# mgp25/OpenLTE

Measured on AMD Instinct MI355X. Metric: DL subframes/sec @20MHz 100RB 64QAM, full chain FFT->CE->demap->rate-unmatch->turbo(REF)->CRC (SURVEY 8d W4), higher is better.
Workload: dtype i8 IQ in, f32 FFT/CE/equaliser, i8 soft bits, i16 path metrics (differences exact modulo 2^16); 1 GPU; W4 full DL chain: 20 MHz/100 RB/64QAM, 9 allocations per subframe (8x12 PRB TBS 3240 + 1x4 PRB TBS 1064), 65536 subframes per GPU, int8 IQ in HBM; subframes_per_gpu=65536, N_ant=1, CFI=2, channel_estimate_form=compact, decoder=REF (reference-faithful, bit-exact), unique_subframes=96, streams_per_gpu=1

## Files before the change

openlte_amd/csrc/turbo.hip:

```cpp
#include <algorithm>
#include <cstring>
#include <initializer_list>
#include <type_traits>
#include <vector>

#include "plan_core.hpp"
#include "turbo_swar.h"

using namespace turbo_geom;

namespace {

constexpr uint32_t RX_NULL_AS_INT = 10000;


__device__ __forceinline__ int sbyte(uint32_t w, int k) { return (int)__builtin_amdgcn_sbfe(w, 8 * k, 8); }

typedef __attribute__((address_space(3))) const uint8_t  lds_u8_t;
typedef __attribute__((address_space(3))) const int8_t   lds_i8_t;
typedef __attribute__((address_space(3))) const uint16_t lds_u16_t;
__device__ __forceinline__ uint32_t lds_u8(uint32_t addr) { return *(lds_u8_t *)(uintptr_t)addr; }
__device__ __forceinline__ int      lds_i8(uint32_t addr) { return *(lds_i8_t *)(uintptr_t)addr; }
__device__ __forceinline__ uint32_t lds_u16(uint32_t addr) { return *(lds_u16_t *)(uintptr_t)addr; }

// ... 967 lines not shown
            }
            if (t < n_t) {
                const uint32_t w = (ch * 64 + t) >> 5, left = n_t - t;
                for (; t < n_t; t += 8) steps8(t);
                decw[(gi * n_w32 + w) * 4 + j] = accv << (32u - left);
            }
        }
        __syncthreads();
    }

#ifdef SMALL_PAD
    if ((padv[0] ^ padv[1] ^ padv[2] ^ padv[3]) == 0x12345678u) decw[0] = 0;
#endif
    uint32_t cur = 0;
    {
        const uint32_t q0 = (uint32_t)__builtin_amdgcn_mov_dpp((int)XY, 0x00, 0xF, 0xF, false), q1 = (uint32_t)__builtin_amdgcn_mov_dpp((int)XY, 0x55, 0xF, 0xF, false);
        const uint32_t q2 = (uint32_t)__builtin_amdgcn_mov_dpp((int)XY, 0xAA, 0xF, 0xF, false), q3 = (uint32_t)__builtin_amdgcn_mov_dpp((int)XY, 0xFF, 0xF, 0xF, false);
        const short pm[8] = {(short)q0, (short)q1, (short)q2, (short)q3, (short)(q0 >> 16), (short)(q1 >> 16), (short)(q2 >> 16), (short)(q3 >> 16)};
        int best = 0;
#pragma unroll
        for (int st = 1; st < 8; st++) {
            const int d = (short)(pm[st] - pm[0]);
            if (d < best) { best = d; cur = st; }
        }
    }

    const uint2 MAP_ID = make_uint2(0x03020100u, 0x07060504u);
    for (uint32_t g = 0; g < n_g; g++) {
        uint32_t       end = (uint32_t)__builtin_amdgcn_readlane((int)cur, (int)(g * 4));
        const uint32_t cb  = mode ? (T0 + g) >> 1 : T0 + g;
        uint32_t      *sgn = pass_of(g).sgn + (seg_off >> 5) + ((size_t)(cb >> 6) * n_chunk * 64 + (cb & 63u)) * 2;
        for (int ch = (int)n_chunk - 1; ch >= 0; ch--) {
            const uint32_t t = (uint32_t)ch * 64 + lane;
            const uint4    w = *reinterpret_cast<const uint4 *>(&decw[(g * n_w32 + (t >> 5)) * 4]);
            const uint32_t sh = 31u - (t & 31u);
            uint2          G = MAP_ID;
            if (t < K) {
                const uint32_t f = 0x06040200u + (((w.x >> sh) & 1u) | ((w.y >> sh) & 1u) << 8 | ((w.z >> sh) & 1u) << 16 | ((w.w >> sh) & 1u) << 24);
                G = make_uint2(f, f);
            }
            G = map_compose(G, map_row_shl<1>(G, MAP_ID));
            G = map_compose(G, map_row_shl<2>(G, MAP_ID));
            G = map_compose(G, map_row_shl<4>(G, MAP_ID));
            G = map_compose(G, map_row_shl<8>(G, MAP_ID));
            const uint32_t row = lane >> 4;
#pragma unroll
            for (int r = 1; r < 4; r++) {
                const uint2 R = make_uint2((uint32_t)__builtin_amdgcn_readlane((int)G.x, 16 * r), (uint32_t)__builtin_amdgcn_readlane((int)G.y, 16 * r));
                if (row < (uint32_t)r) G = map_compose(G, R);
            }
            const uint2    Gn  = make_uint2((uint32_t)__shfl_down((int)G.x, 1u), (uint32_t)__shfl_down((int)G.y, 1u));
            const uint32_t nxt = lane == 63 ? end : map_at(Gn, end);
            const uint32_t st  = map_at(G, end);
            const bool     pos = (nxt < st) || (nxt == st && nxt == 0);
            const uint64_t neg = __ballot(t < K && !pos);
            if (lane == 0) *reinterpret_cast<uint2 *>(sgn + (size_t)ch * 64 * 2) = make_uint2((uint32_t)neg, (uint32_t)(neg >> 32));
            end = (uint32_t)__builtin_amdgcn_readlane((int)st, 0);
        }
    }
}

namespace sw = turbo_swar;
struct UnitWords { uint32_t w[5]; };
__device__ __forceinline__ UnitWords load_unit_words(const uint8_t *arr, size_t tile_off, uint32_t lane, uint32_t u)
{
    const uint4 c    = *reinterpret_cast<const uint4 *>(arr + unit_off(tile_off, lane, u));
    uint32_t    prev = 0x7F7F7F7Fu;
    if (u > 0) prev = *reinterpret_cast<const uint32_t *>(arr + unit_off(tile_off, lane, u - 1) + 12);
    return UnitWords{{prev, c.x, c.y, c.z, c.w}};
}
__device__ __forceinline__ UnitWords load_unit_joined(const uint8_t *mag, const uint32_t *sgn, size_t tile_off, uint32_t lane, uint32_t u)
{
    UnitWords      w = load_unit_words(mag, tile_off, lane, u);
    const uint32_t *sp = sgn + (tile_off >> 5) + ((size_t)(u >> 2) * 64 + lane) * 2;
    const uint2    c = *reinterpret_cast<const uint2 *>(sp);
    uint32_t       ph = 0;
    if ((u & 3u) == 0 && u > 0) ph = sp[1 - 128];
    const uint32_t b = sw::unit_sign_bits(c.x, c.y, ph, u);
    if (u > 0) w.w[0] = sw::joined_from_bits(w.w[0], b & 15u);
#pragma unroll
    for (int j = 0; j < 4; j++) w.w[j + 1] = sw::joined_from_bits(w.w[j + 1], (b >> (4 * j + 4)) & 15u);
    return w;
}
struct PermArgs { const uint8_t *M1; const uint32_t *S1;  const uint8_t *X2; uint8_t *out[2];  };

#ifndef PERM_NB
#define PERM_NB 4
#endif
static_assert(PERM_NB == PERM_BLOCKS, "a size's perm grid is a multiple of 128 workgroups (the merged decode's map granularity) only for four blocks per workgroup");
template <int NSLOT, bool MULTI = false>
__global__ __launch_bounds__(384) void k_turbo_perm(PermArgs a, uint32_t K_arg, uint32_t n_cb_arg, const uint16_t *__restrict__ pi_arg, MultiArgs ma)
{
    static_assert(NSLOT == 1, "one unit per thread");
    uint32_t K = K_arg, n_cb = n_cb_arg, bidx = blockIdx.x, grid = gridDim.x;
    size_t   seg_off = 0;
    const uint16_t *__restrict__ pi = pi_arg;
    if constexpr (MULTI) {
        const_seg_t &sg = multi_seg(ma, blockIdx.x >> 7);
        K = sg.K; n_cb = sg.n_cb; pi = (const uint16_t *)sg.pi; bidx = blockIdx.x - sg.wg_perm; grid = sg.perm_grid;
        seg_off = sg.arr_off;
    }
    extern __shared__ __attribute__((aligned(16))) int8_t smp[];
    int8_t *mtab = smp, *sm = smp + MTAB_N;
    const uint32_t Kp = kpad64(K), n_units = Kp >> 4;
    int           *red_i = reinterpret_cast<int *>(sm + Kp);
    const uint32_t u0 = threadIdx.x;
    const int      nv = (u0 < n_units) ? min(16, max(0, (int)K - 16 * (int)u0)) : -1;
    IdxRaw         praw;
    {
        const uint4 *ip = reinterpret_cast<const uint4 *>(pi + 16 * (size_t)(nv > 0 ? u0 : 0));
        const uint32_t kk = K | K << 16;
        praw.lo = ip[0];
        praw.hi = (nv > 8) ? ip[1] : make_uint4(kk, kk, kk, kk);
    }
#pragma unroll 1
    for (uint32_t it = 0; it < PERM_NB; it++) {
        const uint32_t cb = xcd_cb(bidx + it * grid, n_cb), tile = cb >> 6, lane = cb & 63;
        const size_t   tile_off = seg_off + (size_t)tile * Kp * 64;
        if (cb >= n_cb) {
            if (MULTI && cb < ((n_cb + 63u) & ~63u) && nv >= 0) {
                *reinterpret_cast<uint4 *>(a.out[0] + unit_off(tile_off, lane, u0)) = make_uint4(0, 0, 0, 0);
                *reinterpret_cast<uint4 *>(a.out[1] + unit_off(tile_off, lane, u0)) = make_uint4(0, 0, 0, 0);
            }
            continue;
        }
        uint32_t u = u0;
        asm volatile("" : "+v"(u), "+v"(praw.lo.x), "+v"(praw.lo.y), "+v"(praw.lo.z), "+v"(praw.lo.w), "+v"(praw.hi.x), "+v"(praw.hi.y), "+v"(praw.hi.z), "+v"(praw.hi.w));
        uint4          X2 = make_uint4(0, 0, 0, 0);
        if (nv >= 0) {
            const UnitWords wa = load_unit_joined(a.M1, a.S1, tile_off, lane, u);
            uint32_t        pa = wa.w[0];
            X2 = *reinterpret_cast<const uint4 *>(a.X2 + unit_off(tile_off, lane, u));
            uint32_t c1[4];
#pragma unroll
            for (int j = 0; j < 4; j++) {
                const uint32_t ja = wa.w[j + 1];
                const sw::SM4  A  = sw::unjoin(ja);
                c1[j] = (4 * j < nv) ? sw::to_tc(sw::step3(A, sw::feedback(ja, pa))) : 0u;
                pa    = ja;
            }
            *reinterpret_cast<uint4 *>(sm + 16 * u) = make_uint4(c1[0], c1[1], c1[2], c1[3]);
        }
        __syncthreads();
        uint4 I1 = make_uint4(0, 0, 0, 0);
        if (nv > 0) {
            uint32_t idx[16];
            unpack_idx16(praw, idx);
            I1 = gather16_bytes(MTAB_N, idx);
        }
        if (nv >= 0) *reinterpret_cast<uint4 *>(a.out[0] + unit_off(tile_off, lane, u)) = I1;
        uint32_t w[16], wm = 0;
        if (nv <= 0) X2 = make_uint4(0, 0, 0, 0);
        abs_sum16(X2, I1, w, wm);
        const int   wmax = block_max_i((int)wm, red_i);
        if (wmax == 254 || wmax == 127) {
            uint32_t o[4];
#pragma unroll
            for (int j = 0; j < 4; j++) {
                const uint32_t p = pack4u(w[4 * j], w[4 * j + 1], w[4 * j + 2], w[4 * j + 3]);
                o[j] = wmax == 254 ? (p >> 1) & 0x7F7F7F7Fu : p;
            }
            if (nv >= 0) *reinterpret_cast<uint4 *>(a.out[1] + unit_off(tile_off, lane, u)) = make_uint4(o[0], o[1], o[2], o[3]);
            continue;
        }
        const float W = (float)wmax;
        for (uint32_t t = threadIdx.x; t < MTAB_N; t += blockDim.x) mtab[t] = (int8_t)(int)(127.0f * ((float)t / W));
        __syncthreads();
        if (nv >= 0) *reinterpret_cast<uint4 *>(a.out[1] + unit_off(tile_off, lane, u)) = lookup16(0, w);
        __syncthreads();
    }
}

struct VoteArgs { const uint8_t *X0, *M1, *M2, *M3; const uint32_t *S1, *S2, *S3; };

template <bool GROUP, int NSLOT, bool MULTI = false>
__global__ __launch_bounds__(384) __attribute__((amdgpu_waves_per_eu(6, 8))) void k_turbo_vote(VoteArgs a, uint32_t K_arg, uint32_t n_cb_arg, const uint16_t *__restrict__ inv_arg,
                                                    uint8_t *__restrict__ c_bits, GroupDesc g, MultiArgs ma)
{
    static_assert(NSLOT == 1, "one unit per thread");
    uint32_t K = K_arg, n_cb = n_cb_arg, bidx = blockIdx.x;
    size_t   seg_off = 0;
    const uint16_t *__restrict__ inv = inv_arg;
    if constexpr (MULTI) {
        const_seg_t &sg = multi_seg(ma, blockIdx.x >> 9);
        K = sg.K; n_cb = sg.n_cb; inv = (const uint16_t *)sg.inv2; bidx = blockIdx.x - sg.wg_cb; seg_off = sg.arr_off;
        g.desc += sg.cb_base;
    }
    extern __shared__ __attribute__((aligned(16))) int8_t sm[];
    const uint32_t cb = xcd_cb(bidx, n_cb), tile = cb >> 6, lane = cb & 63, Kp = kpad64(K), n_units = Kp >> 4;
    if (cb >= n_cb) return;
    const size_t   tile_off = seg_off + (size_t)tile * Kp * 64;
    int8_t        *d12 = sm, *bits = sm + 2 * Kp + 32;
    uint32_t      *red_u = reinterpret_cast<uint32_t *>(bits + Kp);
    const uint32_t u  = threadIdx.x;
    const int      nv = (u < n_units) ? min(16, max(0, (int)K - 16 * (int)u)) : -1;
    IdxRaw vraw;
    {
        const uint4 *ip = reinterpret_cast<const uint4 *>(inv + 16 * (size_t)(nv > 0 ? u : 0));
        vraw.lo = ip[0];
        vraw.hi = ip[1];
    }
    const uint32_t crc_w0 = (GROUP && nv > 0) ? g.crc_tab[MI_CRC_TAB_BIAS + K - 16 * u - 16] : 0u;
    v2s            s0e[4], s0o[4];
    if (threadIdx.x == 0) *reinterpret_cast<uint32_t *>(d12 + 2 * Kp) = 0u;
    if (nv >= 0) {
        const UnitWords wa = load_unit_joined(a.M1, a.S1, tile_off, lane, u), wb = load_unit_joined(a.M2, a.S2, tile_off, lane, u),
                        wc = load_unit_joined(a.M3, a.S3, tile_off, lane, u);
        uint32_t        pa = wa.w[0], pb = wb.w[0], pc = wc.w[0];
        const uint4    x0 = *reinterpret_cast<const uint4 *>(a.X0 + unit_off(tile_off, lane, u));
        const uint32_t x0w[4] = {x0.x, x0.y, x0.z, x0.w};
        uint32_t       dn[8];
#pragma unroll
        for (int j = 0; j < 4; j++) {
            const uint32_t ja = wa.w[j + 1], jb = wb.w[j + 1], jc = wc.w[j + 1];
            const sw::SM4  A = sw::unjoin(ja), B = sw::unjoin(jb), B_ = sw::unjoin(jc);
            const sw::SM4  F  = sw::feedback(ja, pa);
            const sw::SM4  G  = sw::feedback(jb, pb);
            const sw::SM4  G_ = sw::feedback(jc, pc);
            pa = ja; pb = jb; pc = jc;
            const uint32_t u1 = sw::step10_biased(A, B, G), n2 = sw::step11_neg_biased(B_, G_);
            const uint32_t de = sw::sub_halves(sw::even_halves(u1), sw::even_halves(n2)), dd = sw::sub_halves(sw::odd_halves(u1), sw::odd_halves(n2));
            const uint32_t x0b = x0w[j] ^ sw::HI, nc = sw::step3_neg_biased(A, F);
            s0e[j] = as_v2s(sw::sub_halves(sw::even_halves(x0b), sw::even_halves(nc)));
            s0o[j] = as_v2s(sw::sub_halves(sw::odd_halves(x0b), sw::odd_halves(nc)));
            const bool in = 4 * j < nv;
            dn[2 * j]     = in ? __builtin_amdgcn_perm(dd, de, 0x05040100u) : 0u;
            dn[2 * j + 1] = in ? __builtin_amdgcn_perm(dd, de, 0x07060302u) : 0u;
        }
        uint4 *dst = reinterpret_cast<uint4 *>(d12 + 32 * u);
        dst[0] = make_uint4(dn[0], dn[1], dn[2], dn[3]);
        dst[1] = make_uint4(dn[4], dn[5], dn[6], dn[7]);
    } else {
#pragma unroll
        for (int j = 0; j < 4; j++) s0e[j] = s0o[j] = (v2s)(0);
    }
    __syncthreads();
    uint32_t alloc = 0, tbs = 0, F = 0, crc = 0;
    if (GROUP) {
        alloc = g.desc[cb].alloc;
        tbs   = g.desc[cb].tbs;
        F     = K - tbs - 24;
    }
    if (nv > 0) {
        const uint32_t  iw[8] = {vraw.lo.x, vraw.lo.y, vraw.lo.z, vraw.lo.w, vraw.hi.x, vraw.hi.y, vraw.hi.z, vraw.hi.w};
        uint32_t        me[4], mo[4], bw[4];
#pragma unroll
        for (int j = 0; j < 4; j++) {
            const uint32_t i0 = iw[2 * j] & 0xFFFFu, i1 = iw[2 * j] >> 16, i2 = iw[2 * j + 1] & 0xFFFFu, i3 = iw[2 * j + 1] >> 16;
            const uint32_t ge = lds_u16(i0) | lds_u16(i2) << 16, go = lds_u16(i1) | lds_u16(i3) << 16;
            me[j] = as_u32((s0e[j] + as_v2s(ge)) >> 15);
            mo[j] = as_u32((s0o[j] + as_v2s(go)) >> 15);
            bw[j] = (me[j] & 0x00010001u) | (mo[j] & 0x00010001u) << 8;
        }
        if (GROUP) {
            if (!(nv == 16 && 16 * u >= F)) {
#pragma unroll
                for (int j = 0; j < 4; j++) {
                    auto ok = [&](int k) { return (k < nv && 16 * u + k >= F) ? 0xFFFFu : 0u; };
                    me[j] &= ok(4 * j) | ok(4 * j + 2) << 16;
                    mo[j] &= ok(4 * j + 1) | ok(4 * j + 3) << 16;
                }
            }
            const uint32_t GS = 0x864CFBu << 8;
            uint32_t       w = crc_w0;
#pragma unroll
            for (int k = 15; k >= 0; k--) {
                const int      j = k >> 2;
                const uint32_t m = (k & 3) == 0 ? (uint32_t)__builtin_amdgcn_sbfe(me[j], 0, 1) : (k & 3) == 1 ? (uint32_t)__builtin_amdgcn_sbfe(mo[j], 0, 1)
                                 : (k & 3) == 2 ? (uint32_t)((int)me[j] >> 31) : (uint32_t)((int)mo[j] >> 31);
                crc ^= w & m;
                if (k > 0) w = (w << 1) ^ ((uint32_t)((int)w >> 31) & GS);
            }
        }
        const uint4 pk = make_uint4(bw[0], bw[1], bw[2], bw[3]);
        if (GROUP) *reinterpret_cast<uint4 *>(bits + 16 * u) = pk;
        else {
            uint2 *o = reinterpret_cast<uint2 *>(c_bits + (size_t)cb * K + 16 * u);
            o[0] = make_uint2(pk.x, pk.y);
            if (nv > 8) o[1] = make_uint2(pk.z, pk.w);
        }
    }
    if (GROUP) {
        crc = wave_xor_u(crc);
        __syncthreads();
        if ((threadIdx.x & 63) == 0) red_u[threadIdx.x >> 6] = crc;
        __syncthreads();
        crc = 0;
        for (uint32_t w = 0; w < (blockDim.x >> 6); w++) crc ^= red_u[w];
        if (threadIdx.x == 0) g.status[alloc] = (crc == 0) ? 0  : 2 ;
        uint8_t *o = g.out_bits + (size_t)alloc * g.out_stride;
        if (g.packed && ((F | tbs) & 7u) == 0) {
            const uint32_t nby = tbs >> 3, nw = nby >> 2;
            auto byte_at = [&](uint32_t m) -> uint32_t {
                const uint2 w = *reinterpret_cast<const uint2 *>(bits + F + 8 * m);
                return (((w.x * 0x08040201u) >> 24) & 0xFu) << 4 | (((w.y * 0x08040201u) >> 24) & 0xFu);
            };
            for (uint32_t m = threadIdx.x; m < nw; m += blockDim.x)
                reinterpret_cast<uint32_t *>(o)[m] = byte_at(4 * m) | byte_at(4 * m + 1) << 8 | byte_at(4 * m + 2) << 16 | byte_at(4 * m + 3) << 24;
            for (uint32_t m = 4 * nw + threadIdx.x; m < nby; m += blockDim.x) o[m] = (uint8_t)byte_at(m);
        } else if (g.packed) {
            for (uint32_t m = threadIdx.x; m < (tbs + 7) >> 3; m += blockDim.x) {
                uint32_t v = 0;
                for (uint32_t b = 0; b < 8; b++) v = v << 1 | ((8 * m + b < tbs) ? ((uint32_t)bits[F + 8 * m + b] & 1u) : 0u);
                o[m] = (uint8_t)v;
            }
        } else if ((F & 3u) == 0) {
            const uint32_t nq = tbs >> 2;
            const uint32_t *bw = reinterpret_cast<const uint32_t *>(bits + F);
            for (uint32_t m = threadIdx.x; m < nq; m += blockDim.x) reinterpret_cast<uint32_t *>(o)[m] = bw[m];
            for (uint32_t m = 4 * nq + threadIdx.x; m < tbs; m += blockDim.x) o[m] = (uint8_t)bits[m + F];
        } else
            for (uint32_t m = threadIdx.x; m < tbs; m += blockDim.x) o[m] = (uint8_t)bits[m + F];
    }
}

__global__ __launch_bounds__(256) void k_cb_desc(GroupDesc g, uint32_t n_cb, const uint32_t *__restrict__ nnn, CbDesc *__restrict__ out)
{
    const uint32_t cb = blockIdx.x * blockDim.x + threadIdx.x;
    if (cb >= n_cb) return;
    const uint32_t a = g.cb_alloc[cb], txm = g.allocs[a].tx_mode;
    const uint32_t combo = g.ul ? 8u + (g.allocs[a].rv_idx & 3u)
                                : ((g.allocs[a].rv_idx & 3u) << 1) | ((txm == 3 || txm == 4 || txm == 8 || txm == 9) ? 1u : 0u);
    CbDesc d;
    d.alloc = a; d.e_off = g.e_off[a]; d.E = g.e_len[a]; d.combo = combo; d.Nnn = nnn[combo];
    d.hard  = (g.allocs[a].mod_type >= 2 && d.E <= d.Nnn) ? 1u : 0u;
    d.tbs   = g.allocs[a].tbs; d.pad = 0;
    out[cb] = d;
}

__global__ __launch_bounds__(256) void k_cb_desc_multi(GroupDesc g, uint32_t n_cb, const KSeg *__restrict__ segs, uint32_t n_seg, CbDesc *__restrict__ out)
{
    const uint32_t cb = blockIdx.x * blockDim.x + threadIdx.x;
    if (cb >= n_cb) return;
    uint32_t lo = 0, hi = n_seg;
    while (hi - lo > 1) {
        const uint32_t mid = (lo + hi) >> 1;
        if (segs[mid].cb_base <= cb) lo = mid; else hi = mid;
    }
    const uint32_t a = g.cb_alloc[cb], txm = g.allocs[a].tx_mode;
    const uint32_t combo = g.ul ? 8u + (g.allocs[a].rv_idx & 3u)
                                : ((g.allocs[a].rv_idx & 3u) << 1) | ((txm == 3 || txm == 4 || txm == 8 || txm == 9) ? 1u : 0u);
    CbDesc d;
    d.alloc = a; d.e_off = g.e_off[a]; d.E = g.e_len[a]; d.combo = combo; d.Nnn = segs[lo].nnn[combo];
    d.hard  = (g.allocs[a].mod_type >= 2 && d.E <= d.Nnn) ? 1u : 0u;
    d.tbs   = g.allocs[a].tbs; d.pad = 0;
    out[cb] = d;
}

__global__ __launch_bounds__(256) void k_rm_rank_table(uint32_t K, uint16_t *__restrict__ tabs, uint32_t *__restrict__ nnn)
{
    const uint32_t combo = blockIdx.y, t = blockIdx.x * blockDim.x + threadIdx.x;
    RmGeom rm;
    if (combo < 8) rm.init(K + 4, (combo & 1) ? 3 : 1, combo >> 1);
    else           rm.init(K + 4, 1, combo - 8, 1, 1, 1, false);
    if (t == 0) nnn[combo] = rm.Nnn;
    if (t >= 3 * K) return;
    const uint32_t x = t / K, i = t - x * K;
    uint32_t p, c;
    rm.pos_cnt(i, (int)x, p, c);
    uint32_t k = 0xFFFFu;
    if (p < rm.N_cb) k = (p >= rm.k0m) ? c - rm.cnt_k0 : rm.Nnn - rm.cnt_k0 + c;
    tabs[(size_t)combo * 3 * K + t] = (uint16_t)k;
}

// ... 542 lines not shown
```

openlte_amd/csrc/turbo_plan.hpp:

```cpp
#pragma once

#include <cstddef>
#include <cstdint>
#include <vector>

#ifdef __HIPCC__
#define MI_HD __host__ __device__
#else
#define MI_HD
#endif
#ifdef __clang__
#define MI_GLOBAL_AS __attribute__((address_space(1)))
#else
#define MI_GLOBAL_AS
#endif

namespace turbo_geom {

MI_HD inline uint32_t kpad64(uint32_t K) { return (K + 63u) & ~63u; }

MI_HD inline uint32_t xcd_chunk(uint32_t n_cb) { return ((((n_cb + 63u) >> 6) + 7u) >> 3) << 6; }
MI_HD inline uint32_t xcd_cb(uint32_t b, uint32_t n_cb) { return (b & 7u) * xcd_chunk(n_cb) + (b >> 3); }
inline uint32_t cb_grid(uint32_t n_cb) { return 8 * xcd_chunk(n_cb); }

constexpr int NCLS = 6;
inline uint32_t cb_width(uint32_t K) { return ((kpad64(K) >> 4) + 63u) & ~63u; }
inline int      cb_class(uint32_t K) { return (int)(cb_width(K) >> 6) - 1; }

constexpr uint32_t PERM_BLOCKS = 4;
inline uint32_t perm_grid_of(uint32_t n_cb) { return ((cb_grid(n_cb) + PERM_BLOCKS - 1) / PERM_BLOCKS + 7u) & ~7u; }

constexpr uint32_t SMALL_G = 8;
inline uint32_t gpw_of(uint32_t n_tr) { return n_tr <= 2048 ? 1u : n_tr <= 4096 ? 2u : n_tr <= 8192 ? 4u : SMALL_G; }
inline size_t   siso_small_lds_bytes(uint32_t gpw, size_t Kp) { return sizeof(uint32_t) * gpw * (64 * 4 * 2 + (Kp >> 5) * 4); }

constexpr uint32_t QTAB_N = 4096;
constexpr uint32_t QTAB_HALF = 2048;
constexpr uint32_t MTAB_N = 256;
constexpr uint32_t PREP_RED_AT = 2 * MTAB_N, PREP_E_AT = PREP_RED_AT + 64, PREP_QTAB_AT = PREP_E_AT, PREP_Q0_AT = PREP_QTAB_AT + QTAB_N;
MI_HD constexpr uint32_t prep_lds_bytes(uint32_t Kp, uint32_t e_cap) { return PREP_E_AT + (e_cap > QTAB_N + Kp ? e_cap : QTAB_N + Kp); }
inline uint32_t stage_cap(uint32_t e_max_bytes) { return (e_max_bytes + 16u + 63u) & ~63u; }
inline bool prep_stages(uint32_t K, uint32_t cap) { return prep_lds_bytes(kpad64(K), cap) <= 48 * 1024; }
inline uint32_t merged_e_cap(uint32_t K, uint32_t e_max_bytes)
{
    const uint32_t cap = stage_cap(e_max_bytes), cap_w = (uint32_t)((15 * (size_t)(K + 4) / 4 + 64 + 63) & ~(size_t)63);
    return prep_stages(K, cap) ? (kpad64(K) <= 1024 ? (cap < cap_w ? cap : cap_w) : cap) : cap_w;
}

inline bool mi_turbo_ref_multi_takes(uint32_t K, uint32_t e_max_bytes) { return (e_max_bytes + (3 * K - 81) - 1) / (3 * K - 81) <= 258; }

constexpr int    N_BYTE_ARRAYS = 8;
constexpr size_t CB_DESC_BYTES = 32;
inline size_t ref_scratch_bytes(size_t arr_bytes, size_t n_slots) { return N_BYTE_ARRAYS * arr_bytes + 3 * (arr_bytes / 2) + 3 * (arr_bytes / 8) + ((n_slots + 63) & ~(size_t)63) * CB_DESC_BYTES; }

}

struct MiKGroup { uint32_t K, n_cb, cb_base, e_max; };

struct KSeg {
    uint32_t        K, n_cb, cb_base, n_tiles;
    uint32_t        wg_cb;
    uint32_t        wg_perm, perm_grid;
    uint32_t        e_cap;
    uint32_t        wv1, wv23;
    uint64_t        arr_off;
    MI_GLOBAL_AS const uint16_t *pi, *inv2, *tabs;
    MI_GLOBAL_AS const uint32_t *nnn;
    uint32_t        ws1, ws23;
    uint64_t        pad;
};
static_assert(sizeof(KSeg) == 96, "KSeg is read with scalar loads: keep it a multiple of 16 bytes");
struct MultiArgs { const KSeg *segs; const uint32_t *map; };

struct MiMultiGeom {
    uint64_t arr_bytes = 0;
    uint32_t n_slots = 0, n_wv1 = 0, n_wv23 = 0;
    uint32_t grid_cb[6] = {0}, grid_perm[6] = {0}, lds_prep[6] = {0}, kp_max[6] = {0};
    uint32_t map_cb[6] = {0}, map_perm[6] = {0}, map_wv1 = 0, map_wv23 = 0;
    uint32_t ord_wv1 = 0, ord_wv23 = 0, n_ord1 = 0, n_ord23 = 0;
    uint32_t siso_pad1 = 0, siso_pad23 = 0;
    int      one_size[6] = {-1, -1, -1, -1, -1, -1};
    uint64_t off_one[6] = {0}; uint32_t e_cap_one[6] = {0};
    uint32_t map_ws1 = 0, map_ws23 = 0, n_ws1 = 0, n_ws23 = 0, gpw1 = 1, gpw23 = 1, kp_all = 0;
    size_t   map_off = 0;
};

struct MiMultiPlan { std::vector<KSeg> segs; std::vector<uint32_t> map; MiMultiGeom geom; };
int mi_turbo_multi_plan(const MiKGroup *groups, uint32_t n_groups, MiMultiPlan *out, const char **err);
```

openlte_amd/csrc/turbo_swar.h:

```cpp
#pragma once

#include <cstdint>

#ifdef __HIPCC__
#define SWAR_FN __host__ __device__ __forceinline__
#else
#define SWAR_FN inline
#endif

namespace turbo_swar {

constexpr uint32_t HI = 0x80808080u, LO7 = 0x7F7F7F7Fu, ONES = 0x01010101u, EVEN = 0x00FF00FFu;

SWAR_FN uint32_t alignbit(uint32_t hi, uint32_t lo, uint32_t sh)
{
#if defined(__HIP_DEVICE_COMPILE__)
    return __builtin_amdgcn_alignbit(hi, lo, sh);
#else
    return (uint32_t)((((uint64_t)hi << 32) | lo) >> sh);
#endif
}
SWAR_FN uint32_t sub_halves(uint32_t a, uint32_t b)
{
#if defined(__HIP_DEVICE_COMPILE__)
    typedef short v2s_t __attribute__((ext_vector_type(2)));
    return __builtin_bit_cast(uint32_t, __builtin_bit_cast(v2s_t, a) - __builtin_bit_cast(v2s_t, b));
#else
    return ((a - (b & 0xFFFFu)) & 0xFFFFu) | ((a & 0xFFFF0000u) - (b & 0xFFFF0000u));
#endif
}

struct SM4 { uint32_t m, s; };

SWAR_FN uint32_t low7(uint32_t bits) { return bits - (bits >> 7); }

SWAR_FN uint32_t to_joined(uint32_t w)
{
    const uint32_t s = w & HI, t = s >> 7;
    return (w ^ (s - t)) + t;
}
SWAR_FN uint32_t joined_from(uint32_t m, uint32_t neg_mask) { return m | (neg_mask & (m + LO7) & HI); }
SWAR_FN uint32_t joined_from_bits(uint32_t m, uint32_t nib) { return m | ((nib * 0x10204080u) & (m + LO7) & HI); }
SWAR_FN uint32_t unit_sign_bits(uint32_t c_lo, uint32_t c_hi, uint32_t prev_hi, uint32_t u)
{
    const uint32_t q = u & 3u;
    const uint64_t c = ((uint64_t)c_hi << 32) | c_lo;
    return q ? (uint32_t)(c >> (16u * q - 4u)) & 0xFFFFFu : (c_lo & 0xFFFFu) << 4 | prev_hi >> 28;
}
SWAR_FN SM4 unjoin(uint32_t j) { return SM4{j & LO7, j & HI}; }
SWAR_FN SM4 split(uint32_t w) { return unjoin(to_joined(w)); }
SWAR_FN uint32_t join(const SM4 &a) { return a.m | a.s; }
SWAR_FN uint32_t to_tc(const SM4 &a)
{
    const uint32_t t = a.s >> 7;
    return ((a.m ^ (a.s - t)) + t) | a.s;
}

SWAR_FN uint32_t biased(uint32_t x, uint32_t neg)
{
    const uint32_t t = neg >> 7;
    return ((x ^ (neg - t)) + t) + (neg ^ HI);
}
SWAR_FN uint32_t even_halves(uint32_t w) { return w & EVEN; }
SWAR_FN uint32_t odd_halves(uint32_t w) { return (w >> 8) & EVEN; }

SWAR_FN uint32_t half_sum(uint32_t ma, uint32_t mb) { return ((ma + mb) >> 1) & LO7; }
SWAR_FN SM4 soft_xor(const SM4 &a, const SM4 &b)
{
    const uint32_t m = half_sum(a.m, b.m);
    return SM4{m, (a.s ^ b.s) & (m + LO7) & HI};
}

SWAR_FN uint32_t delay2(uint32_t cur, uint32_t prev) { return alignbit(cur, prev, 16); }
SWAR_FN uint32_t delay3(uint32_t cur, uint32_t prev) { return alignbit(cur, prev, 8); }
SWAR_FN SM4 feedback(uint32_t cur_joined, uint32_t prev_joined)
{
    const uint32_t d2 = delay2(cur_joined, prev_joined), d3 = delay3(cur_joined, prev_joined);
    const uint32_t x = d2 ^ d3;
    const uint32_t m = (d2 & d3 & LO7) + ((x >> 1) & 0x3F3F3F3Fu);
    return SM4{m, x & (m + LO7) & HI};
}

SWAR_FN SM4 step3(const SM4 &A, const SM4 &F) { return soft_xor(A, F); }
SWAR_FN uint32_t step3_neg_biased(const SM4 &A, const SM4 &F) { return biased(half_sum(A.m, F.m), A.s ^ F.s ^ HI); }

SWAR_FN uint32_t avg_biased(uint32_t xb, uint32_t yb) { return (xb & yb) + (((xb ^ yb) >> 1) & LO7); }

SWAR_FN uint32_t step10_biased(const SM4 &A, const SM4 &B, const SM4 &G)
{
    const uint32_t mx = B.s ^ G.s, tm = mx >> 7, m7 = mx - tm;
    const uint32_t y  = (A.m & m7) | (B.m & ~m7);
    const uint32_t w  = avg_biased(G.m | HI, biased(y, mx & (A.s ^ B.s)));
    return (w ^ (m7 | mx)) + tm;
}
SWAR_FN uint32_t step11_neg_biased(const SM4 &B, const SM4 &G)
{
    const uint32_t mx = B.s ^ G.s, tm = mx >> 7, m7 = mx - tm;
    const uint32_t w  = avg_biased(B.m | HI, biased(G.m, mx & B.s));
    return (w ^ ~(m7 | mx)) + (tm ^ ONES);
}

SWAR_FN uint32_t traceback_entry(uint32_t byte, uint32_t cur)
{
    uint32_t sgn = 0;
    for (int k = 0; k < 2; k++) {
        const uint32_t nib = k ? byte >> 4 : byte & 15u;
        const uint32_t j = cur & 3u, bit = (nib >> (3 - j)) & 1u, st = 2 * j + bit;
        const bool     pos = (cur < st) || (cur == st && cur == 0);
        if (!pos) sgn |= k ? 1u << 30 : 1u << 31;
        cur = st;
    }
    return cur | sgn;
}

}
```

Baseline: 2.888 million subframes/s.

## Spread tail-wave work across lanes with per-wave word width in perm and vote

The perm and vote kernels used to give each thread one 16-byte unit, so in the last partially filled wave many lanes sat idle while a few did four words of work. Each wave now picks a words-per-lane width (4, 2 or 1) from how full its tail is, and the per-lane code is templated on that width. Partially filled tail waves therefore spread their units across more lanes with shorter per-lane chains. In exchange there are three code paths per kernel, more sign-bit extraction arithmetic, and narrower memory accesses in the tail waves.

```diff
diff --git a/openlte_amd/csrc/turbo.hip b/openlte_amd/csrc/turbo.hip
--- a/openlte_amd/csrc/turbo.hip
+++ b/openlte_amd/csrc/turbo.hip
@@ -1073,12 +1073,168 @@
     for (int j = 0; j < 4; j++) w.w[j + 1] = sw::joined_from_bits(w.w[j + 1], (b >> (4 * j + 4)) & 15u);
     return w;
 }
+
+template <int N> __device__ __forceinline__ void load_words(const void *p, uint32_t (&w)[N])
+{
+    static_assert(N == 1 || N == 2 || N == 4 || N == 8, "");
+    if constexpr (N == 1) w[0] = *reinterpret_cast<const uint32_t *>(p);
+    else if constexpr (N == 2) { const uint2 v = *reinterpret_cast<const uint2 *>(p); w[0] = v.x; w[1] = v.y; }
+    else {
+#pragma unroll
+        for (int h = 0; h < N / 4; h++) { const uint4 v = reinterpret_cast<const uint4 *>(p)[h]; w[4 * h] = v.x; w[4 * h + 1] = v.y; w[4 * h + 2] = v.z; w[4 * h + 3] = v.w; }
+    }
+}
+template <int N> __device__ __forceinline__ void store_words(void *p, const uint32_t (&w)[N])
+{
+    static_assert(N == 1 || N == 2 || N == 4 || N == 8, "");
+    if constexpr (N == 1) *reinterpret_cast<uint32_t *>(p) = w[0];
+    else if constexpr (N == 2) *reinterpret_cast<uint2 *>(p) = make_uint2(w[0], w[1]);
+    else {
+#pragma unroll
+        for (int h = 0; h < N / 4; h++) reinterpret_cast<uint4 *>(p)[h] = make_uint4(w[4 * h], w[4 * h + 1], w[4 * h + 2], w[4 * h + 3]);
+    }
+}
+template <int W> struct LaneAt { uint32_t u, j0, p0; int nv; };
+template <int W> __device__ __forceinline__ LaneAt<W> lane_at(uint32_t K, uint32_t n_units, uint32_t wave )
+{
+    LaneAt<W> l;
+    bool      live;
+    if constexpr (W == 4) { l.u = threadIdx.x; l.j0 = 0; live = l.u < n_units; }
+    else { const LaneWords lw = lane_words(n_units, wave, threadIdx.x & 63u, W); l.u = lw.unit; l.j0 = lw.word; live = lw.live; }
+    l.p0 = 16 * l.u + 4 * l.j0;
+    l.nv = live ? min(4 * W, max(0, (int)K - (int)l.p0)) : -1;
+    return l;
+}
+template <int W> struct LaneW { uint32_t w[W + 1]; };
+template <int W> __device__ __forceinline__ LaneW<W> load_lane_joined(const uint8_t *mag, const uint32_t *sgn, size_t tile_off, uint32_t lane, uint32_t u, uint32_t j0)
+{
+    LaneW<W> r;
+    if constexpr (W == 4) {
+        const UnitWords w = load_unit_joined(mag, sgn, tile_off, lane, u);
+#pragma unroll
+        for (int j = 0; j < 5; j++) r.w[j] = w.w[j];
+    } else {
+        uint32_t       cur[W];
+        const uint32_t g = 4 * u + j0;
+        load_words<W>(mag + unit_off(tile_off, lane, u) + 4 * j0, cur);
+        uint32_t prev = 0x7F7F7F7Fu;
+        if (g > 0) prev = *reinterpret_cast<const uint32_t *>(mag + unit_off(tile_off, lane, (g - 1) >> 2) + 4 * ((g - 1) & 3u));
+        const uint32_t *sp = sgn + (tile_off >> 5) + ((size_t)(u >> 2) * 64 + lane) * 2;
+        const uint2    c = *reinterpret_cast<const uint2 *>(sp);
+        uint32_t       ph = 0;
+        if ((g & 15u) == 0 && g > 0) ph = sp[1 - 128];
+        const uint32_t b = sw::word_sign_bits(c.x, c.y, ph, g & 15u, W);
+        r.w[0] = g > 0 ? sw::joined_from_bits(prev, b & 15u) : prev;
+#pragma unroll
+        for (int j = 0; j < W; j++) r.w[j + 1] = sw::joined_from_bits(cur[j], (b >> (4 * j + 4)) & 15u);
+    }
+    return r;
+}
 struct PermArgs { const uint8_t *M1; const uint32_t *S1;  const uint8_t *X2; uint8_t *out[2];  };
 
 #ifndef PERM_NB
 #define PERM_NB 4
 #endif
 static_assert(PERM_NB == PERM_BLOCKS, "a size's perm grid is a multiple of 128 workgroups (the merged decode's map granularity) only for four blocks per workgroup");
+template <bool MULTI, int W>
+__device__ __forceinline__ void perm_lane(const PermArgs &a, uint32_t K, uint32_t n_cb, uint32_t bidx, uint32_t grid, size_t seg_off, const uint16_t *__restrict__ pi,
+                                          int8_t *mtab, int8_t *sm, int *red_i, uint32_t wave)
+{
+    const uint32_t  Kp = kpad64(K);
+    const LaneAt<W> l = lane_at<W>(K, Kp >> 4, wave);
+    const int       nv = l.nv;
+    uint32_t        praw[2 * W];
+    {
+        const uint32_t kk = K | K << 16;
+        if constexpr (W == 4) {
+            const uint4 *ip = reinterpret_cast<const uint4 *>(pi + 16 * (size_t)(nv > 0 ? l.u : 0));
+            const uint4 lo = ip[0], hi = (nv > 8) ? ip[1] : make_uint4(kk, kk, kk, kk);
+            praw[0] = lo.x; praw[1] = lo.y; praw[2] = lo.z; praw[3] = lo.w; praw[4] = hi.x; praw[5] = hi.y; praw[6] = hi.z; praw[7] = hi.w;
+        } else {
+            load_words<2 * W>(pi + (nv > 0 ? l.p0 : 0), praw);
+            if (nv <= 0) {
+#pragma unroll
+                for (int j = 0; j < 2 * W; j++) praw[j] = kk;
+            }
+        }
+    }
+#pragma unroll 1
+    for (uint32_t it = 0; it < PERM_NB; it++) {
+        const uint32_t cb = xcd_cb(bidx + it * grid, n_cb), tile = cb >> 6, lane = cb & 63;
+        const size_t   tile_off = seg_off + (size_t)tile * Kp * 64;
+        if (cb >= n_cb) {
+            if (MULTI && cb < ((n_cb + 63u) & ~63u) && nv >= 0) {
+                const uint32_t z[W] = {};
+                store_words<W>(a.out[0] + unit_off(tile_off, lane, l.u) + 4 * l.j0, z);
+                store_words<W>(a.out[1] + unit_off(tile_off, lane, l.u) + 4 * l.j0, z);
+            }
+            continue;
+        }
+        uint32_t u = l.u, j0 = l.j0;
+        if constexpr (W == 4) asm volatile("" : "+v"(u), "+v"(praw[0]), "+v"(praw[1]), "+v"(praw[2]), "+v"(praw[3]), "+v"(praw[4]), "+v"(praw[5]), "+v"(praw[6]), "+v"(praw[7]));
+        else if constexpr (W == 2) asm volatile("" : "+v"(u), "+v"(j0), "+v"(praw[0]), "+v"(praw[1]), "+v"(praw[2]), "+v"(praw[3]));
+        else asm volatile("" : "+v"(u), "+v"(j0), "+v"(praw[0]), "+v"(praw[1]));
+        const size_t at = unit_off(tile_off, lane, u) + 4 * j0;
+        uint32_t     X2[W] = {};
+        if (nv >= 0) {
+            const LaneW<W> wa = load_lane_joined<W>(a.M1, a.S1, tile_off, lane, u, j0);
+            uint32_t       pa = wa.w[0];
+            load_words<W>(a.X2 + at, X2);
+            uint32_t c1[W];
+#pragma unroll
+            for (int j = 0; j < W; j++) {
+                const uint32_t ja = wa.w[j + 1];
+                const sw::SM4  A  = sw::unjoin(ja);
+                c1[j] = (4 * j < nv) ? sw::to_tc(sw::step3(A, sw::feedback(ja, pa))) : 0u;
+                pa    = ja;
+            }
+            store_words<W>(sm + 16 * u + 4 * j0, c1);
+        }
+        __syncthreads();
+        uint32_t I1[W] = {};
+        if (nv > 0) {
+#pragma unroll
+            for (int j = 0; j < W; j++) {
+                const uint32_t i01 = praw[2 * j], i23 = praw[2 * j + 1];
+                I1[j] = pack4u(lds_u8(MTAB_N + (i01 & 0xFFFFu)), lds_u8(MTAB_N + (i01 >> 16)), lds_u8(MTAB_N + (i23 & 0xFFFFu)), lds_u8(MTAB_N + (i23 >> 16)));
+            }
+        }
+        if (nv >= 0) store_words<W>(a.out[0] + at, I1);
+        uint32_t w[4 * W], wm = 0;
+        if (nv <= 0) {
+#pragma unroll
+            for (int j = 0; j < W; j++) X2[j] = 0u;
+        }
+#pragma unroll
+        for (int j = 0; j < W; j++) {
+            const uint32_t xb = bias4(X2[j]), ib = bias4(I1[j]);
+            w[4 * j]     = abs_sum2<0>(xb, ib);
+            w[4 * j + 1] = abs_sum2<1>(xb, ib);
+            w[4 * j + 2] = abs_sum2<2>(xb, ib);
+            w[4 * j + 3] = abs_sum2<3>(xb, ib);
+            wm = max(max(wm, w[4 * j]), max(w[4 * j + 1], max(w[4 * j + 2], w[4 * j + 3])));
+        }
+        const int   wmax = block_max_i((int)wm, red_i);
+        uint32_t    o[W];
+        if (wmax == 254 || wmax == 127) {
+#pragma unroll
+            for (int j = 0; j < W; j++) {
+                const uint32_t p = pack4u(w[4 * j], w[4 * j + 1], w[4 * j + 2], w[4 * j + 3]);
+                o[j] = wmax == 254 ? (p >> 1) & 0x7F7F7F7Fu : p;
+            }
+            if (nv >= 0) store_words<W>(a.out[1] + at, o);
+            continue;
+        }
+        const float Wf = (float)wmax;
+        for (uint32_t t = threadIdx.x; t < MTAB_N; t += blockDim.x) mtab[t] = (int8_t)(int)(127.0f * ((float)t / Wf));
+        __syncthreads();
+#pragma unroll
+        for (int j = 0; j < W; j++) o[j] = pack4u(lds_u8(w[4 * j]), lds_u8(w[4 * j + 1]), lds_u8(w[4 * j + 2]), lds_u8(w[4 * j + 3]));
+        if (nv >= 0) store_words<W>(a.out[1] + at, o);
+        __syncthreads();
+    }
+}
+
 template <int NSLOT, bool MULTI = false>
 __global__ __launch_bounds__(384) void k_turbo_perm(PermArgs a, uint32_t K_arg, uint32_t n_cb_arg, const uint16_t *__restrict__ pi_arg, MultiArgs ma)
 {
@@ -1093,76 +1249,105 @@
     }
     extern __shared__ __attribute__((aligned(16))) int8_t smp[];
     int8_t *mtab = smp, *sm = smp + MTAB_N;
-    const uint32_t Kp = kpad64(K), n_units = Kp >> 4;
+    const uint32_t Kp = kpad64(K);
     int           *red_i = reinterpret_cast<int *>(sm + Kp);
-    const uint32_t u0 = threadIdx.x;
-    const int      nv = (u0 < n_units) ? min(16, max(0, (int)K - 16 * (int)u0)) : -1;
-    IdxRaw         praw;
-    {
-        const uint4 *ip = reinterpret_cast<const uint4 *>(pi + 16 * (size_t)(nv > 0 ? u0 : 0));
-        const uint32_t kk = K | K << 16;
-        praw.lo = ip[0];
-        praw.hi = (nv > 8) ? ip[1] : make_uint4(kk, kk, kk, kk);
-    }
-#pragma unroll 1
-    for (uint32_t it = 0; it < PERM_NB; it++) {
-        const uint32_t cb = xcd_cb(bidx + it * grid, n_cb), tile = cb >> 6, lane = cb & 63;
-        const size_t   tile_off = seg_off + (size_t)tile * Kp * 64;
-        if (cb >= n_cb) {
-            if (MULTI && cb < ((n_cb + 63u) & ~63u) && nv >= 0) {
-                *reinterpret_cast<uint4 *>(a.out[0] + unit_off(tile_off, lane, u0)) = make_uint4(0, 0, 0, 0);
-                *reinterpret_cast<uint4 *>(a.out[1] + unit_off(tile_off, lane, u0)) = make_uint4(0, 0, 0, 0);
-            }
-            continue;
-        }
-        uint32_t u = u0;
-        asm volatile("" : "+v"(u), "+v"(praw.lo.x), "+v"(praw.lo.y), "+v"(praw.lo.z), "+v"(praw.lo.w), "+v"(praw.hi.x), "+v"(praw.hi.y), "+v"(praw.hi.z), "+v"(praw.hi.w));
-        uint4          X2 = make_uint4(0, 0, 0, 0);
-        if (nv >= 0) {
-            const UnitWords wa = load_unit_joined(a.M1, a.S1, tile_off, lane, u);
-            uint32_t        pa = wa.w[0];
-            X2 = *reinterpret_cast<const uint4 *>(a.X2 + unit_off(tile_off, lane, u));
-            uint32_t c1[4];
-#pragma unroll
-            for (int j = 0; j < 4; j++) {
-                const uint32_t ja = wa.w[j + 1];
-                const sw::SM4  A  = sw::unjoin(ja);
-                c1[j] = (4 * j < nv) ? sw::to_tc(sw::step3(A, sw::feedback(ja, pa))) : 0u;
-                pa    = ja;
-            }
-            *reinterpret_cast<uint4 *>(sm + 16 * u) = make_uint4(c1[0], c1[1], c1[2], c1[3]);
-        }
-        __syncthreads();
-        uint4 I1 = make_uint4(0, 0, 0, 0);
-        if (nv > 0) {
-            uint32_t idx[16];
-            unpack_idx16(praw, idx);
-            I1 = gather16_bytes(MTAB_N, idx);
-        }
-        if (nv >= 0) *reinterpret_cast<uint4 *>(a.out[0] + unit_off(tile_off, lane, u)) = I1;
-        uint32_t w[16], wm = 0;
-        if (nv <= 0) X2 = make_uint4(0, 0, 0, 0);
-        abs_sum16(X2, I1, w, wm);
-        const int   wmax = block_max_i((int)wm, red_i);
-        if (wmax == 254 || wmax == 127) {
-            uint32_t o[4];
-#pragma unroll
-            for (int j = 0; j < 4; j++) {
-                const uint32_t p = pack4u(w[4 * j], w[4 * j + 1], w[4 * j + 2], w[4 * j + 3]);
-                o[j] = wmax == 254 ? (p >> 1) & 0x7F7F7F7Fu : p;
-            }
-            if (nv >= 0) *reinterpret_cast<uint4 *>(a.out[1] + unit_off(tile_off, lane, u)) = make_uint4(o[0], o[1], o[2], o[3]);
-            continue;
-        }
-        const float W = (float)wmax;
-        for (uint32_t t = threadIdx.x; t < MTAB_N; t += blockDim.x) mtab[t] = (int8_t)(int)(127.0f * ((float)t / W));
-        __syncthreads();
-        if (nv >= 0) *reinterpret_cast<uint4 *>(a.out[1] + unit_off(tile_off, lane, u)) = lookup16(0, w);
-        __syncthreads();
-    }
+    const uint32_t wave = (uint32_t)__builtin_amdgcn_readfirstlane((int)(threadIdx.x >> 6)), nw = wave_words(Kp >> 4, wave);
+    if (nw == 4) perm_lane<MULTI, 4>(a, K, n_cb, bidx, grid, seg_off, pi, mtab, sm, red_i, wave);
+    else if (nw == 2) perm_lane<MULTI, 2>(a, K, n_cb, bidx, grid, seg_off, pi, mtab, sm, red_i, wave);
+    else perm_lane<MULTI, 1>(a, K, n_cb, bidx, grid, seg_off, pi, mtab, sm, red_i, wave);
 }
 
 struct VoteArgs { const uint8_t *X0, *M1, *M2, *M3; const uint32_t *S1, *S2, *S3; };
+
+template <bool GROUP, int W>
+__device__ __forceinline__ uint32_t vote_lane(const VoteArgs &a, const GroupDesc &g, uint32_t K, uint32_t cb, size_t tile_off, const uint16_t *__restrict__ inv,
+                                              uint8_t *__restrict__ c_bits, int8_t *d12, int8_t *bits, uint32_t wave, uint32_t &alloc, uint32_t &tbs, uint32_t &F)
+{
+    const uint32_t  Kp = kpad64(K), lane = cb & 63;
+    const LaneAt<W> l = lane_at<W>(K, Kp >> 4, wave);
+    const uint32_t  u = l.u, j0 = l.j0, p0 = l.p0;
+    const int       nv = l.nv;
+    uint32_t iw[2 * W];
+    load_words<2 * W>(inv + (nv > 0 ? p0 : 0), iw);
+    const uint32_t crc_w0 = (GROUP && nv > 0) ? g.crc_tab[MI_CRC_TAB_BIAS + K - p0 - 4 * W] : 0u;
+    v2s            s0e[W], s0o[W];
+    if (threadIdx.x == 0) *reinterpret_cast<uint32_t *>(d12 + 2 * Kp) = 0u;
+    if (nv >= 0) {
+        const LaneW<W> wa = load_lane_joined<W>(a.M1, a.S1, tile_off, lane, u, j0), wb = load_lane_joined<W>(a.M2, a.S2, tile_off, lane, u, j0),
+                       wc = load_lane_joined<W>(a.M3, a.S3, tile_off, lane, u, j0);
+        uint32_t       pa = wa.w[0], pb = wb.w[0], pc = wc.w[0];
+        uint32_t       x0w[W];
+        load_words<W>(a.X0 + unit_off(tile_off, lane, u) + 4 * j0, x0w);
+        uint32_t       dn[2 * W];
+#pragma unroll
+        for (int j = 0; j < W; j++) {
+            const uint32_t ja = wa.w[j + 1], jb = wb.w[j + 1], jc = wc.w[j + 1];
+            const sw::SM4  A = sw::unjoin(ja), B = sw::unjoin(jb), B_ = sw::unjoin(jc);
+            const sw::SM4  Fa = sw::feedback(ja, pa);
+            const sw::SM4  G  = sw::feedback(jb, pb);
+            const sw::SM4  G_ = sw::feedback(jc, pc);
+            pa = ja; pb = jb; pc = jc;
+            const uint32_t u1 = sw::step10_biased(A, B, G), n2 = sw::step11_neg_biased(B_, G_);
+            const uint32_t de = sw::sub_halves(sw::even_halves(u1), sw::even_halves(n2)), dd = sw::sub_halves(sw::odd_halves(u1), sw::odd_halves(n2));
+            const uint32_t x0b = x0w[j] ^ sw::HI, nc = sw::step3_neg_biased(A, Fa);
+            s0e[j] = as_v2s(sw::sub_halves(sw::even_halves(x0b), sw::even_halves(nc)));
+            s0o[j] = as_v2s(sw::sub_halves(sw::odd_halves(x0b), sw::odd_halves(nc)));
+            const bool in = 4 * j < nv;
+            dn[2 * j]     = in ? __builtin_amdgcn_perm(dd, de, 0x05040100u) : 0u;
+            dn[2 * j + 1] = in ? __builtin_amdgcn_perm(dd, de, 0x07060302u) : 0u;
+        }
+        store_words<2 * W>(d12 + 2 * p0, dn);
+    } else {
+#pragma unroll
+        for (int j = 0; j < W; j++) s0e[j] = s0o[j] = (v2s)(0);
+    }
+    __syncthreads();
+    uint32_t crc = 0;
+    if (GROUP) {
+        alloc = g.desc[cb].alloc;
+        tbs   = g.desc[cb].tbs;
+        F     = K - tbs - 24;
+    }
+    if (nv > 0) {
+        uint32_t        me[W], mo[W], bw[W];
+#pragma unroll
+        for (int j = 0; j < W; j++) {
+            const uint32_t i0 = iw[2 * j] & 0xFFFFu, i1 = iw[2 * j] >> 16, i2 = iw[2 * j + 1] & 0xFFFFu, i3 = iw[2 * j + 1] >> 16;
+            const uint32_t ge = lds_u16(i0) | lds_u16(i2) << 16, go = lds_u16(i1) | lds_u16(i3) << 16;
+            me[j] = as_u32((s0e[j] + as_v2s(ge)) >> 15);
+            mo[j] = as_u32((s0o[j] + as_v2s(go)) >> 15);
+            bw[j] = (me[j] & 0x00010001u) | (mo[j] & 0x00010001u) << 8;
+        }
+        if (GROUP) {
+            if (!(nv == 4 * W && p0 >= F)) {
+#pragma unroll
+                for (int j = 0; j < W; j++) {
+                    auto ok = [&](int k) { return (k < nv && p0 + k >= F) ? 0xFFFFu : 0u; };
+                    me[j] &= ok(4 * j) | ok(4 * j + 2) << 16;
+                    mo[j] &= ok(4 * j + 1) | ok(4 * j + 3) << 16;
+                }
+            }
+            const uint32_t GS = 0x864CFBu << 8;
+            uint32_t       w = crc_w0;
+#pragma unroll
+            for (int k = 4 * W - 1; k >= 0; k--) {
+                const int      j = k >> 2;
+                const uint32_t m = (k & 3) == 0 ? (uint32_t)__builtin_amdgcn_sbfe(me[j], 0, 1) : (k & 3) == 1 ? (uint32_t)__builtin_amdgcn_sbfe(mo[j], 0, 1)
+                                 : (k & 3) == 2 ? (uint32_t)((int)me[j] >> 31) : (uint32_t)((int)mo[j] >> 31);
+                crc ^= w & m;
+                if (k > 0) w = (w << 1) ^ ((uint32_t)((int)w >> 31) & GS);
+            }
+        }
+        if (GROUP) store_words<W>(bits + p0, bw);
+        else if constexpr (W == 4) {
+            uint2 *o = reinterpret_cast<uint2 *>(c_bits + (size_t)cb * K + 16 * u);
+            o[0] = make_uint2(bw[0], bw[1]);
+            if (nv > 8) o[1] = make_uint2(bw[2], bw[3]);
+        } else
+            store_words<W>(c_bits + (size_t)cb * K + p0, bw);
+    }
+    return crc;
+}
 
 template <bool GROUP, int NSLOT, bool MULTI = false>
 __global__ __launch_bounds__(384) __attribute__((amdgpu_waves_per_eu(6, 8))) void k_turbo_vote(VoteArgs a, uint32_t K_arg, uint32_t n_cb_arg, const uint16_t *__restrict__ inv_arg,
@@ -1178,99 +1363,16 @@
         g.desc += sg.cb_base;
     }
     extern __shared__ __attribute__((aligned(16))) int8_t sm[];
-    const uint32_t cb = xcd_cb(bidx, n_cb), tile = cb >> 6, lane = cb & 63, Kp = kpad64(K), n_units = Kp >> 4;
+    const uint32_t cb = xcd_cb(bidx, n_cb), tile = cb >> 6, Kp = kpad64(K);
     if (cb >= n_cb) return;
     const size_t   tile_off = seg_off + (size_t)tile * Kp * 64;
     int8_t        *d12 = sm, *bits = sm + 2 * Kp + 32;
     uint32_t      *red_u = reinterpret_cast<uint32_t *>(bits + Kp);
-    const uint32_t u  = threadIdx.x;
-    const int      nv = (u < n_units) ? min(16, max(0, (int)K - 16 * (int)u)) : -1;
-    IdxRaw vraw;
-    {
-        const uint4 *ip = reinterpret_cast<const uint4 *>(inv + 16 * (size_t)(nv > 0 ? u : 0));
-        vraw.lo = ip[0];
-        vraw.hi = ip[1];
-    }
-    const uint32_t crc_w0 = (GROUP && nv > 0) ? g.crc_tab[MI_CRC_TAB_BIAS + K - 16 * u - 16] : 0u;
-    v2s            s0e[4], s0o[4];
-    if (threadIdx.x == 0) *reinterpret_cast<uint32_t *>(d12 + 2 * Kp) = 0u;
-    if (nv >= 0) {
-        const UnitWords wa = load_unit_joined(a.M1, a.S1, tile_off, lane, u), wb = load_unit_joined(a.M2, a.S2, tile_off, lane, u),
-                        wc = load_unit_joined(a.M3, a.S3, tile_off, lane, u);
-        uint32_t        pa = wa.w[0], pb = wb.w[0], pc = wc.w[0];
-        const uint4    x0 = *reinterpret_cast<const uint4 *>(a.X0 + unit_off(tile_off, lane, u));
-        const uint32_t x0w[4] = {x0.x, x0.y, x0.z, x0.w};
-        uint32_t       dn[8];
-#pragma unroll
-        for (int j = 0; j < 4; j++) {
-            const uint32_t ja = wa.w[j + 1], jb = wb.w[j + 1], jc = wc.w[j + 1];
-            const sw::SM4  A = sw::unjoin(ja), B = sw::unjoin(jb), B_ = sw::unjoin(jc);
-            const sw::SM4  F  = sw::feedback(ja, pa);
-            const sw::SM4  G  = sw::feedback(jb, pb);
-            const sw::SM4  G_ = sw::feedback(jc, pc);
-            pa = ja; pb = jb; pc = jc;
-            const uint32_t u1 = sw::step10_biased(A, B, G), n2 = sw::step11_neg_biased(B_, G_);
-            const uint32_t de = sw::sub_halves(sw::even_halves(u1), sw::even_halves(n2)), dd = sw::sub_halves(sw::odd_halves(u1), sw::odd_halves(n2));
-            const uint32_t x0b = x0w[j] ^ sw::HI, nc = sw::step3_neg_biased(A, F);
-            s0e[j] = as_v2s(sw::sub_halves(sw::even_halves(x0b), sw::even_halves(nc)));
-            s0o[j] = as_v2s(sw::sub_halves(sw::odd_halves(x0b), sw::odd_halves(nc)));
-            const bool in = 4 * j < nv;
-            dn[2 * j]     = in ? __builtin_amdgcn_perm(dd, de, 0x05040100u) : 0u;
-            dn[2 * j + 1] = in ? __builtin_amdgcn_perm(dd, de, 0x07060302u) : 0u;
-        }
-        uint4 *dst = reinterpret_cast<uint4 *>(d12 + 32 * u);
-        dst[0] = make_uint4(dn[0], dn[1], dn[2], dn[3]);
-        dst[1] = make_uint4(dn[4], dn[5], dn[6], dn[7]);
-    } else {
-#pragma unroll
-        for (int j = 0; j < 4; j++) s0e[j] = s0o[j] = (v2s)(0);
-    }
-    __syncthreads();
-    uint32_t alloc = 0, tbs = 0, F = 0, crc = 0;
-    if (GROUP) {
-        alloc = g.desc[cb].alloc;
-        tbs   = g.desc[cb].tbs;
-        F     = K - tbs - 24;
-    }
-    if (nv > 0) {
-        const uint32_t  iw[8] = {vraw.lo.x, vraw.lo.y, vraw.lo.z, vraw.lo.w, vraw.hi.x, vraw.hi.y, vraw.hi.z, vraw.hi.w};
-        uint32_t        me[4], mo[4], bw[4];
-#pragma unroll
-        for (int j = 0; j < 4; j++) {
-            const uint32_t i0 = iw[2 * j] & 0xFFFFu, i1 = iw[2 * j] >> 16, i2 = iw[2 * j + 1] & 0xFFFFu, i3 = iw[2 * j + 1] >> 16;
-            const uint32_t ge = lds_u16(i0) | lds_u16(i2) << 16, go = lds_u16(i1) | lds_u16(i3) << 16;
-            me[j] = as_u32((s0e[j] + as_v2s(ge)) >> 15);
-            mo[j] = as_u32((s0o[j] + as_v2s(go)) >> 15);
-            bw[j] = (me[j] & 0x00010001u) | (mo[j] & 0x00010001u) << 8;
-        }
-        if (GROUP) {
-            if (!(nv == 16 && 16 * u >= F)) {
-#pragma unroll
-                for (int j = 0; j < 4; j++) {
-                    auto ok = [&](int k) { return (k < nv && 16 * u + k >= F) ? 0xFFFFu : 0u; };
-                    me[j] &= ok(4 * j) | ok(4 * j + 2) << 16;
-                    mo[j] &= ok(4 * j + 1) | ok(4 * j + 3) << 16;
-                }
-            }
-            const uint32_t GS = 0x864CFBu << 8;
-            uint32_t       w = crc_w0;
-#pragma unroll
-            for (int k = 15; k >= 0; k--) {
-                const int      j = k >> 2;
-                const uint32_t m = (k & 3) == 0 ? (uint32_t)__builtin_amdgcn_sbfe(me[j], 0, 1) : (k & 3) == 1 ? (uint32_t)__builtin_amdgcn_sbfe(mo[j], 0, 1)
-                                 : (k & 3) == 2 ? (uint32_t)((int)me[j] >> 31) : (uint32_t)((int)mo[j] >> 31);
-                crc ^= w & m;
-                if (k > 0) w = (w << 1) ^ ((uint32_t)((int)w >> 31) & GS);
-            }
-        }
-        const uint4 pk = make_uint4(bw[0], bw[1], bw[2], bw[3]);
-        if (GROUP) *reinterpret_cast<uint4 *>(bits + 16 * u) = pk;
-        else {
-            uint2 *o = reinterpret_cast<uint2 *>(c_bits + (size_t)cb * K + 16 * u);
-            o[0] = make_uint2(pk.x, pk.y);
-            if (nv > 8) o[1] = make_uint2(pk.z, pk.w);
-        }
-    }
+    const uint32_t wave = (uint32_t)__builtin_amdgcn_readfirstlane((int)(threadIdx.x >> 6)), nw = wave_words(Kp >> 4, wave);
+    uint32_t       alloc = 0, tbs = 0, F = 0, crc;
+    if (nw == 4) crc = vote_lane<GROUP, 4>(a, g, K, cb, tile_off, inv, c_bits, d12, bits, wave, alloc, tbs, F);
+    else if (nw == 2) crc = vote_lane<GROUP, 2>(a, g, K, cb, tile_off, inv, c_bits, d12, bits, wave, alloc, tbs, F);
+    else crc = vote_lane<GROUP, 1>(a, g, K, cb, tile_off, inv, c_bits, d12, bits, wave, alloc, tbs, F);
     if (GROUP) {
         crc = wave_xor_u(crc);
         __syncthreads();
diff --git a/openlte_amd/csrc/turbo_plan.hpp b/openlte_amd/csrc/turbo_plan.hpp
--- a/openlte_amd/csrc/turbo_plan.hpp
+++ b/openlte_amd/csrc/turbo_plan.hpp
@@ -26,6 +26,19 @@
 constexpr int NCLS = 6;
 inline uint32_t cb_width(uint32_t K) { return ((kpad64(K) >> 4) + 63u) & ~63u; }
 inline int      cb_class(uint32_t K) { return (int)(cb_width(K) >> 6) - 1; }
+
+MI_HD inline uint32_t tail_words(uint32_t n_units)
+{
+    const uint32_t r = n_units & 63u;
+    return (r == 0 || r > 32) ? 4u : r > 16 ? 2u : 1u;
+}
+MI_HD inline uint32_t wave_words(uint32_t n_units, uint32_t wave) { return wave == (n_units >> 6) ? tail_words(n_units) : 4u; }
+struct LaneWords { uint32_t unit, word; bool live; };
+MI_HD inline LaneWords lane_words(uint32_t n_units, uint32_t wave, uint32_t lane, uint32_t words)
+{
+    const uint32_t q = lane * words, unit = wave * 64u + (q >> 2);
+    return LaneWords{unit, q & 3u, unit < n_units};
+}
 
 constexpr uint32_t PERM_BLOCKS = 4;
 inline uint32_t perm_grid_of(uint32_t n_cb) { return ((cb_grid(n_cb) + PERM_BLOCKS - 1) / PERM_BLOCKS + 7u) & ~7u; }
diff --git a/openlte_amd/csrc/turbo_swar.h b/openlte_amd/csrc/turbo_swar.h
--- a/openlte_amd/csrc/turbo_swar.h
+++ b/openlte_amd/csrc/turbo_swar.h
@@ -46,6 +46,12 @@
     const uint32_t q = u & 3u;
     const uint64_t c = ((uint64_t)c_hi << 32) | c_lo;
     return q ? (uint32_t)(c >> (16u * q - 4u)) & 0xFFFFFu : (c_lo & 0xFFFFu) << 4 | prev_hi >> 28;
+}
+SWAR_FN uint32_t word_sign_bits(uint32_t c_lo, uint32_t c_hi, uint32_t prev_hi, uint32_t g, uint32_t nw)
+{
+    const uint64_t c = ((uint64_t)c_hi << 32) | c_lo;
+    const uint32_t mask = (16u << (4u * nw)) - 1u;
+    return g ? (uint32_t)(c >> (4u * g - 4u)) & mask : ((c_lo << 4) & mask) | prev_hi >> 28;
 }
 SWAR_FN SM4 unjoin(uint32_t j) { return SM4{j & LO7, j & HI}; }
 SWAR_FN SM4 split(uint32_t w) { return unjoin(to_joined(w)); }
```

After: 2.903 million subframes/s (median of 6 runs). About the same (+0.5%).
